# tomn681/Flow-Matching-and-Diffusion-Models

Measured on AMD Instinct MI355X. Metric: train images/sec + sampler steps/sec, LDCT 256x256 UNet at 1/2/4/8 MI355X, higher is better.
Workload: dtype bf16; 1 GPU; LDCT 2D 256x256 flow-matching train step (configs/flow_matching/ldct_flow_matching.json, EfficientUNetND 113M, concatenate conditioning) + 50-step FlowMatchEuler sampler; global_batch=8, per_gpu_batch=8, img=256, parallelism=dp1, hipgraph=True

## Files before the change

flow-matching-and-diffusion-models_amd/csrc/conv.hip:

```cpp
#include <cstdlib>
#include "halo_args.h"
#include "splitk_combine.h"

namespace {

struct KArgs {
  fmd_conv_desc d;
  fmd_gn_apply_desc g;
  int M;
  int T;
  int C;
  int nk1;
  int nk;
  int per_split;
  int ntp, ntc;
  int stats_rows;
  int par;
  int Mfull;
  int pack;
};

template <int BCO, int BPX, int WM, int WN, int BK, bool GNA = false>
__global__ __launch_bounds__(256, 2) void conv_igemm(const KArgs A) {
  constexpr int NT = 256;
// ... 352 lines not shown
#pragma unroll
      for (int kk = 0; kk < NB; ++kk) {
        const int k = kk;
        const int pi = (tid + 256 * (k0 + kk)) / CHT;
        const int p = min(px0 + pi, A.M - 1);
        vz[k] = *(const u32x4*)((const bf16r*)g.dz + (size_t)p * C + co);
        vx[k] = first ? *(const u32x4*)((const bf16r*)g.x0 + (size_t)p * C0 + co)
                      : *(const u32x4*)((const bf16r*)g.x1 + (size_t)p * C1 + (co - C0));
        old[k] = u32x4{0u, 0u, 0u, 0u};
        if (accf)
          old[k] = first ? *(const u32x4*)((const bf16r*)g.dx0 + (size_t)p * C0 + co)
                         : *(const u32x4*)((const bf16r*)g.dx1 + (size_t)p * C1 + (co - C0));
      }
#pragma unroll
      for (int k = 0; k < NB; ++k) {
        const int pi = (tid + 256 * (k0 + k)) / CHT;
        const int p = px0 + pi;
        if (p >= A.M) continue;
        const int n = p / HWo;
        const u32x4 ve = *(const u32x4*)(tile + pi * BCO + ((c16 ^ (pi & (CHT - 1))) * 8));
        bf16r* dst = first ? (bf16r*)g.dx0 + (size_t)p * C0 + co : (bf16r*)g.dx1 + (size_t)p * C1 + (co - C0);
        const float* pp = g.P + (size_t)n * C + co;
        const float* qq = g.Q + (size_t)n * C + co;
        const float* rr = g.R + (size_t)n * C + co;
        const f32x4 P0 = *(const f32x4*)pp, P1 = *(const f32x4*)(pp + 4);
        const f32x4 Q0 = *(const f32x4*)qq, Q1 = *(const f32x4*)(qq + 4);
        const f32x4 R0 = *(const f32x4*)rr, R1 = *(const f32x4*)(rr + 4);
        const float Pv[8] = {P0[0], P0[1], P0[2], P0[3], P1[0], P1[1], P1[2], P1[3]};
        const float Qv[8] = {Q0[0], Q0[1], Q0[2], Q0[3], Q1[0], Q1[1], Q1[2], Q1[3]};
        const float Rv[8] = {R0[0], R0[1], R0[2], R0[3], R1[0], R1[1], R1[2], R1[3]};
        u32x4 o;
#pragma unroll
        for (int e = 0; e < 4; ++e) {
          float lo = Pv[2 * e] * bf_lo(vz[k][e]) + Qv[2 * e] * bf_lo(vx[k][e]) + Rv[2 * e] + bf_lo(ve[e]);
          float hi = Pv[2 * e + 1] * bf_hi(vz[k][e]) + Qv[2 * e + 1] * bf_hi(vx[k][e]) + Rv[2 * e + 1] +
                     bf_hi(ve[e]);
          if (accf) { lo += bf_lo(old[k][e]); hi += bf_hi(old[k][e]); }
          o[e] = pack2(lo, hi);
        }
        *(u32x4*)dst = o;
      }
      }
    }
    return;
  }

  const bool stats = d.stats != nullptr;
  const bool dep = d.ep_a != nullptr;
  const bool hasx = d.ep_x0 != nullptr;
  float st1[TM][4], st2[TM][4];
#pragma unroll
  for (int i = 0; i < TM; ++i)
#pragma unroll
    for (int r = 0; r < 4; ++r) { st1[i][r] = 0.f; st2[i][r] = 0.f; }

#pragma unroll
  for (int i = 0; i < TM; ++i) {
    const int co = co0 + wm * (BCO / WM) + 16 * i + 4 * lq;
    if (co >= K) continue;
    const bool full = co + 3 < K;
    float bias[4] = {0.f, 0.f, 0.f, 0.f};
    if (d.bias) {
      for (int r = 0; r < 4; ++r) bias[r] = (co + r < K) ? d.bias[co + r] : 0.f;
    }
    if (d.bias2) {
      for (int r = 0; r < 4; ++r) bias[r] += (co + r < K) ? d.bias2[co + r] : 0.f;
    }
#pragma unroll
    for (int j = 0; j < TN; ++j) {
// ... 581 lines not shown
```

flow-matching-and-diffusion-models_amd/csrc/wgrad.hip:

```cpp
#include "common.h"
#include "../../include/fmdiff.h"

namespace {

constexpr int BCO = 128, BCI = 128, BKP = 32;

struct WArgs {
  fmd_wgrad_desc d;
  int M, T, C, ntc, nci, per_split, nsteps, ldy;
  int merged;
};

FMD_DEV int swz(int row) { return 4 * ((row & 3) | (((row >> 3) & 1) << 2)); }
FMD_DEV int lds_off(int row, int unit) { return row * 128 + 4 * (unit ^ swz(row)); }

FMD_DEV void wgrad_body(const WArgs& A, int bx, const int split, const int nsplit) {
  __shared__ __attribute__((aligned(16))) bf16r lds[2][2][BKP * 128];
  __shared__ float bsum[4][BCO];
  const fmd_wgrad_desc& d = A.d;
  const int tid = threadIdx.x, lane = tid & 63, wid = tid >> 6;
  const int wm = wid >> 1, wn = wid & 1;

  const int tco = bx % A.ntc; bx /= A.ntc;
  const int tci = bx % A.nci; bx /= A.nci;
// ... 406 lines not shown
    rc = (int)hipGetLastError();
  }
  if (rc) return rc;
  int nblk = 0;
  for (int j = 0; j < n; ++j) {
    const WArgs& A = G.a[j];
    const int lanes = 512 / (16 * A.T);
    G.gx[j] = max(1, min(G.nsplit[j], lanes));
    G.start[j] = nblk;
    int rows = A.d.K;
    if (G.nsplit[j] == 1) {
      G.gx[j] = lanes;
      rows = (A.d.K + lanes - 1) / lanes;
    }
    nblk += rows * ((A.C + RC - 1) / RC);
  }
  for (int j = n; j <= FMD_WGRAD_GROUP_MAX; ++j) G.start[j] = nblk;
  hipLaunchKernelGGL(wgrad_reduce2_group, dim3(nblk), dim3(512), 0, s, G);
  return (int)hipGetLastError();
}

extern "C" int fmd_wgrad(const fmd_wgrad_desc* d, fmd_stream_t stream) {
  hipStream_t s = (hipStream_t)stream;
  if (int rc = check_desc(d)) return rc;
  WArgs A = make_args(d);
  const int splits = d->splits > 1 ? d->splits : 1;
  int rc = d->force_generic ? 1 : fmd_wgrad_halo(d, stream);
  if (rc == 1) {
    dim3 grid(A.ntc * (A.merged ? A.nci : A.nci * A.T), splits);
    hipLaunchKernelGGL(wgrad_kernel, grid, dim3(256), 0, s, A);
    rc = (int)hipGetLastError();
  }
  if (rc) return rc;
  if (A.T > 27) return -4;
  if (A.C % 4 == 0) {
    const int sl = max(1, min(splits, 512 / (16 * A.T)));
    hipLaunchKernelGGL(wgrad_reduce2, dim3(d->K, (A.C + RC - 1) / RC), dim3(512), 0, s, A, splits, splits, 1, sl);
  } else {
    hipLaunchKernelGGL(wgrad_reduce, dim3(d->K, (A.C + RC - 1) / RC), dim3(256), 0, s, A, splits, splits, 1);
  }
  return (int)hipGetLastError();
}
```

flow-matching-and-diffusion-models_amd/fmdiff/_lib.py:

```python
from __future__ import annotations

import ctypes as C
import os

LIB_PATH = os.environ.get("FMD_LIB") or os.path.join(os.path.dirname(os.path.abspath(__file__)), "lib",
                                                     "libfmdiff_hip.so")

p = C.c_void_p
i32 = C.c_int32
i64 = C.c_int64
f32 = C.c_float
u32 = C.c_uint32


class ConvDesc(C.Structure):
    _fields_ = [
        ("N", i32), ("Hs", i32), ("Ws", i32), ("C0", i32), ("C1", i32), ("Ho", i32), ("Wo", i32), ("K", i32),
        ("ks", i32), ("stride", i32), ("pad", i32), ("upsample", i32), ("transposed", i32),
        ("src0", p), ("src1", p), ("pro_a", p), ("pro_b", p), ("pro_silu", i32), ("wgt", p),
        ("src2", p), ("src3", p), ("C2", i32), ("C3", i32), ("wgt2", p),
        ("bias", p), ("bias2", p), ("bias_nc", p), ("resid", p), ("out", p), ("out_f32", i32), ("accumulate", i32),
        ("stats", p), ("ep_x0", p), ("ep_x1", p), ("ep_C0", i32), ("ep_a", p), ("ep_b", p),
        ("ws", p), ("splits", i32), ("force_generic", i32), ("wgt_tiled", p), ("wgt2_tiled", p),
        ("Ds", i32), ("Do", i32), ("gout", p),
        ("fold_st0", p), ("fold_rows0", i32), ("fold_st1", p), ("fold_rows1", i32), ("fold_G", i32),
        ("fold_eps", f32), ("fold_gamma", p), ("fold_beta", p), ("fold_emb", p), ("fold_emb_stride", i32),
        ("tickets", p), ("n_tickets", i32), ("tickets_rows", i32),
    ]


class ConvPlan(C.Structure):
    _fields_ = [("kernel", i32), ("tile_rows", i32), ("bco", i32), ("bpx", i32), ("tickets", i32),
                ("combine_launch", i32), ("stats_rows", i32), ("fold", i32)]


CONV_IGEMM, CONV_HALO8, CONV_HALO9 = 1, 2, 3
CONV_TICKET_HALO, CONV_TICKET_IGEMM, CONV_WANT_STATS = 1, 2, 4


class WgradDesc(C.Structure):
    _fields_ = [
        ("N", i32), ("Hs", i32), ("Ws", i32), ("C0", i32), ("C1", i32), ("Ho", i32), ("Wo", i32), ("K", i32),
        ("ks", i32), ("stride", i32), ("pad", i32), ("upsample", i32),
        ("src0", p), ("src1", p), ("pro_a", p), ("pro_b", p), ("pro_silu", i32), ("dy", p), ("ldy", i32), ("dw", p), ("db", p),
        ("accumulate", i32), ("ws", p), ("splits", i32), ("force_generic", i32), ("Ds", i32), ("Do", i32),
    ]


class GnApplyDesc(C.Structure):
    _fields_ = [
        ("dz", p), ("x0", p), ("x1", p), ("C0", i32), ("P", p), ("Q", p), ("R", p),
        ("dx0", p), ("acc0", i32), ("dx1", p), ("acc1", i32),
    ]


class GnOutDesc(C.Structure):
    _fields_ = [("G", i32), ("eps", f32), ("gamma", p), ("beta", p), ("emb", p), ("emb_stride", i32),
                ("emb_mode", i32), ("silu", i32), ("a", p), ("b", p), ("mean_rstd", p), ("t", p)]


class ConvSmallDesc(C.Structure):
    _fields_ = [
        ("N", i32), ("Hs", i32), ("Ws", i32), ("C0", i32), ("C1", i32), ("Ho", i32), ("Wo", i32), ("K", i32),
        ("mode", i32), ("src0", p), ("src1", p), ("wgt", p), ("st0", p), ("rows0", i32), ("st1", p), ("rows1", i32),
        ("G", i32), ("eps", f32), ("gamma", p), ("beta", p), ("emb", p), ("emb_stride", i32), ("silu", i32),
        ("src2", p), ("src3", p), ("C2", i32), ("C3", i32), ("wgt2", p), ("bias", p), ("bias2", p), ("bias_nc", p),
        ("bias_nc_stride", i32), ("resid", p),
        ("out", p), ("stats", p), ("part", p), ("part_bytes", i64), ("tickets", p), ("n_tickets", i32), ("split", i32),
    ]


LINCOMB_MAX = 6


class LincombDesc(C.Structure):
    _fields_ = [("out", p), ("in_", p * LINCOMB_MAX), ("c", C.c_float * LINCOMB_MAX), ("nin", i32), ("n", i64)]


SCHED_NCOEF = 12


class SchedStepDesc(C.Structure):
    _fields_ = [("x", p), ("eps", p), ("ring", p * 4), ("last", p), ("coef", p), ("index", p), ("N", i32), ("Cx", i32),
                ("HW", i32), ("Kpad", i32), ("cond", p), ("Cc", i32), ("Cpad", i32), ("next", p)]


class GbJob(C.Structure):
    _fields_ = [("ws", p), ("dgamma", p), ("dbeta", p), ("N", i32), ("C", i32)]


GB_MAX = 64


class VqPlan(C.Structure):
    _fields_ = [("splits", i32), ("block_rows", i32), ("tile_codes", i32), ("codes_per_split", i32), ("Kpad", i32),
                ("Dpad", i32), ("finalize_rows", i32)]


SIGNATURES = {
    "fmd_conv": [C.POINTER(ConvDesc), p],
    "fmd_conv_plan": [C.POINTER(ConvDesc), i32, C.POINTER(ConvPlan)],
    "fmd_conv_halo": [C.POINTER(ConvDesc), p],
    "fmd_conv_gn_apply": [C.POINTER(ConvDesc), C.POINTER(GnApplyDesc), p],
    "fmd_conv_gn": [C.POINTER(ConvDesc), C.POINTER(GnOutDesc), p],
    "fmd_wgrad": [C.POINTER(WgradDesc), p],
    "fmd_wgrad_workspace": [C.POINTER(WgradDesc)],
    "fmd_wgrad_halo": [C.POINTER(WgradDesc), p],
    "fmd_wgrad_group": [C.POINTER(WgradDesc), i32, p],
    "fmd_wgrad_halo_group": [C.POINTER(WgradDesc), i32, p],
    "fmd_halo_tiled_size": [i32, i32, i32],
    "fmd_tile_weights_halo": [p, i32, i32, i32, p, p],
    "fmd_conv_s2d": [C.POINTER(ConvDesc), p],
    "fmd_conv_d2s": [C.POINTER(ConvDesc), p],
    "fmd_conv_small_plan": [C.POINTER(ConvSmallDesc)],
    "fmd_conv_small_split": [C.POINTER(ConvSmallDesc)],
    "fmd_conv_small": [C.POINTER(ConvSmallDesc), p],
    "fmd_s2d_tiled_size": [i32, i32, i32],
    "fmd_s2d_tile_weights": [p, i32, i32, i32, i32, p, p],
    "fmd_s2d_tiled_size_nd": [i32, i32, i32, i32, i32],
    "fmd_s2d_tile_weights_nd": [p, i32, i32, i32, i32, i32, p, p],
    "fmd_channel_stats": [p, p, p, i32, i32, i32, i32, i32, p, p],
    "fmd_stats_fold": [p, i64, i32, i32, p, p],
    "fmd_gn_prep": [p, i32, p, i32, i32, i32, i32, i32, i32, f32, p, p, p, i32, i32, p, p, p, p],
    "fmd_gn_bwd_prep": [p, i32, i32, i32, i32, i32, p, p, p, p, i32, i32, p, p, p, p, p, p, i32, p, i32, p, p],
    "fmd_gn_apply_fwd": [p, p, i32, i32, i64, i32, p, p, i32, p, p],
    "fmd_gn_fused_apply": [p, p, i32, i32, i32, i32, i32, f32, p, p, p, i32, i32, i32, p, p, p, p, p],
    "fmd_dropout_apply": [p, i32, i64, i32, f32, p, u32, p, p, p, p, p],
    "fmd_gn_gb_fold": [p, i32, p],
    "fmd_lincomb": [C.POINTER(LincombDesc), p],
    "fmd_sched_step": [C.POINTER(SchedStepDesc), p],
    "fmd_halo_set_min_workgroups": [i32],
    "fmd_halo_set_th8_max_workgroups": [i32],
    "fmd_halo_set_th4_max_workgroups": [i32],
    "fmd_conv_gn_set_block_channels": [i32],
    "fmd_gn_bwd_apply": [p, p, p, i32, i32, i64, i32, p, p, p, p, p, i32, p, i32, p],
    "fmd_prep_weights": [p, i32, i32, i32, i32, i32, i32, p, p],
    "fmd_prep_weights_t": [p, i32, i32, i32, i32, i32, i32, p, p],
    "fmd_prep_weights_batch": [p, i32, i32, p],
    "fmd_prep_weights_batch_cubic": [p, i32, i32, p],
    "fmd_nchw_to_nhwc": [p, i32, i32, i32, i32, p, p],
    "fmd_nhwc_to_nchw": [p, i32, i32, i32, i32, i32, p, p],
    "fmd_sum_pool2": [p, i32, i32, i32, i32, p, i32, p],
# ... 96 lines not shown
```

flow-matching-and-diffusion-models_amd/fmdiff/runtime/engine.py:

```python
from __future__ import annotations

import math
import weakref
from typing import List, Optional, Tuple

import torch

from . import ops, tuning
from ..nn.blocks.attention import DiffusersAttentionND, SpatialCrossAttention, SpatialSelfAttention
from ..nn.blocks.residual import ResBlockND
from ..nn.ops.convolution import ConvND
from ..nn.ops.upsampling import DownsampleND, UpsampleND
from ..nn.params import Conv, Identity

BF16 = torch.bfloat16
F32 = torch.float32
CPAD = 8
HALO_BK = 32
MAT3D = bool(tuning.get("MAT3D"))
DEPTH_HALO = bool(tuning.get("DEPTH_HALO"))
S2D_HALO = bool(tuning.get("S2D_HALO"))
S2D_3D = S2D_HALO and bool(tuning.get("S2D_3D"))
POINT_1X1 = bool(tuning.get("POINT_1X1"))
SMALL_ATTN = bool(tuning.get("SMALL_ATTN"))
# ... 546 lines not shown
            a2, b2, mr2 = ops.gn_prep(hst, None, N, HW, Cout, 0, g2.num_groups, g2.eps, g2.weight, g2.bias)
        pf2 = (dict(st0=hst, groups=g2.num_groups, eps=g2.eps, gamma=g2.weight, beta=g2.bias, emb=eo if ss else None,
                    emb_stride=es if ss else 0) if a2 is None and t2 is None else None)
        sk = m.skip_connection
        kw = {}
        if isinstance(sk, Identity):
            if x1 is not None:
                raise ValueError("identity skip with concatenated input")
            kw["resid"] = x0.t
        else:
            _check_conv(sk.conv, 1, 1, 0)
        if mat2 and not halo2:
            halo2 = self._halo_ok(N, sp, Cout, Cout)
        if not isinstance(sk, Identity):
            s2, s2t = self._wts(sk.conv.weight, 0, halo2)
            kw.update(src2=x0.t, src3=x1.t if x1 else None, wgt2=s2, wgt2_tiled=s2t, bias2=sk.conv.bias)
        point2 = POINT_1X1 and sp == (1, 1) and c2.weight.dim() == 4 and not halo2
        w2, w2t = (self.wc.get(self.wc.center(c2.weight), 0), None) if point2 else self._wts(c2.weight, 0, halo2)
        if point2:
            kw.update(ks=1, pad=0)
        if mat2 and t2 is None:
            t2 = ops.gn_apply_fwd(h, None, a2, b2)
        if drop:
            ops.dropout_apply(t2, drop, seed, salt, out=t2)
        gg2 = (torch.empty_like(h) if keep_g and t2 is None and halo2 and not point2 and Cout % HALO_BK == 0
               else None)
        out, ost = ops.conv(t2 if t2 is not None else h, Cout, w2,
                            pro=None if (t2 is not None or pf2 is not None) else (a2, b2, True), pro_fold=pf2,
                            bias=c2.bias, want_stats="free", wgt_tiled=w2t, gout=gg2, **kw)
        o = Act(out, ost)
        if ctx.tape is None:
            return o

        def bwd():
            dy = o.grad

            def wg2():
                if t2 is not None or gg2 is not None:
                    ops.wgrad(t2 if t2 is not None else gg2, dy, c2.weight.grad, db=c2.bias.grad)
                else:
                    ops.wgrad(h, dy, c2.weight.grad, pro=(a2, b2, True), db=c2.bias.grad)
                if not isinstance(sk, Identity):
                    ops.wgrad(x0.t, dy, sk.conv.weight.grad, src1=x1.t if x1 else None, ks=1, pad=0,
                              db=sk.conv.bias.grad)
            self._wg(wg2, N * HW)
            extra = dy if isinstance(sk, Identity) else None
            if drop:
                dd, _ = self.dgrad3x3(c2.weight, dy, Cout, sp)
                dz2 = ops.dropout_apply(dd, drop, seed, salt, ep=(h, a2, b2), out=dd)
                s2 = ops.channel_stats(dz2, y=(h, None, Cout))
            else:
                dz2, s2 = self.dgrad3x3(c2.weight, dy, Cout, sp, ep=(h, None, a2, b2), want_stats=True)
            if slot is not None:
                demb, ds_ = ctx.demb_all[:, slot[0]:slot[0] + slot[1]], self.gl.total
            elif eo is not None:
                demb = torch.empty_like(eo)
                ds_ = demb.shape[1]
            else:
                demb, ds_ = None, 0
            if ss:
                P2, Q2, R2 = ops.gn_bwd_prep(s2, N, HW, Cout, g2.num_groups, mr2, g2.weight, g2.bias, g2.weight.grad,
                                             g2.bias.grad, emb=eo, emb_stride=es, emb_mode=1, demb=demb,
                                             demb_stride=ds_)
            elif add:
                P2, Q2, R2 = ops.gn_bwd_prep(s2, N, HW, Cout, g2.num_groups, mr2, g2.weight, g2.bias, g2.weight.grad,
                                             g2.bias.grad, emb_mode=2, demb=demb, demb_stride=ds_, fwd=hst)
            else:
                P2, Q2, R2 = ops.gn_bwd_prep(s2, N, HW, Cout, g2.num_groups, mr2, g2.weight, g2.bias, g2.weight.grad,
                                             g2.bias.grad)
            dh = torch.empty_like(h)
            ops.gn_bwd_apply(dz2, h, None, P2, Q2, R2, None, dh, 0)
            del dz2
            if t1 is not None or gg1 is not None:
                self._wg(lambda: ops.wgrad(t1 if t1 is not None else gg1, dh, c1.weight.grad, db=c1.bias.grad),
                         N * HW)
            else:
                self._wg(lambda: ops.wgrad(x0.t, dh, c1.weight.grad, src1=x1.t if x1 else None, pro=(a1, b1, True),
                                           db=c1.bias.grad), N * HW)
            dz1, s1 = self.dgrad3x3(c1.weight, dh, Cin, sp, ep=(x0.t, x1.t if x1 else None, a1, b1),
                                    want_stats=True)
            P1, Q1, R1 = ops.gn_bwd_prep(s1, N, HW, Cin, g1.num_groups, mr1, g1.weight, g1.bias, g1.weight.grad,
                                         g1.bias.grad)
            d0, acc0 = _gdest(x0)
            d1, acc1 = _gdest(x1)
            if isinstance(sk, Identity):
                ops.gn_bwd_apply(dz1, x0.t, x1.t if x1 else None, P1, Q1, R1, extra, d0, acc0, d1, acc1)
            else:
                ops.conv1x1_gn_apply(dy, self.wc.get(sk.conv.weight, 1), dz1, x0.t, x1.t if x1 else None,
                                     P1, Q1, R1, d0, acc0, d1, acc1)
            if (ss or add) and slot is None:
                ops.linear_bwd(ctx.emb, el.weight, demb, el.weight.grad, el.bias.grad, dx=ctx.demb, dx_acc=True,
                               in_silu=m.emb_activation_before_proj)
        ctx.tape.append(bwd)
        return o

    def _res_block_small(self, m: ResBlockND, x0: Act, x1: Optional[Act], eo, es, ss: bool, add: bool):
        N, H, W, C0 = x0.t.shape
        C1 = x1.C if x1 is not None else 0
        Cout = m.out_channels
        c1, c2 = m.conv1.conv, m.conv2.conv
        if c1.weight.dim() != 4 or c2.weight.dim() != 4:
            return None
        _check_conv(c1, 3, 1, 1)
        _check_conv(c2, 3, 1, 1)
        point = POINT_1X1 and (H, W) == (1, 1)
        mode = "point" if point else "s1"
        g1, g2 = m.norm1, m.norm2
        sk = m.skip_connection
        ident = isinstance(sk, Identity)
        if ident and x1 is not None:
            raise ValueError("identity skip with concatenated input")
        if not ident:
            _check_conv(sk.conv, 1, 1, 0)
        rows = 64 if (H * W) % 64 == 0 else H * W

        def probe(a):
            return a.stats if a.stats is not None else ops.Stats(None, rows)
        gn1 = dict(st0=probe(x0), st1=probe(x1) if x1 is not None else None, groups=g1.num_groups, eps=g1.eps)
        gn2 = dict(st0=ops.Stats(None, rows), groups=g2.num_groups, eps=g2.eps, emb=eo if ss else None,
# ... 514 lines not shown
```

flow-matching-and-diffusion-models_amd/fmdiff/runtime/ops.py:

```python
from __future__ import annotations

import ctypes as C
from dataclasses import dataclass
from typing import Optional, Tuple

import torch

from .. import _lib
from . import tuning, wgrad_plan
from .._lib import ConvDesc, GnApplyDesc, GnOutDesc, WgradDesc

BF16 = torch.bfloat16
F32 = torch.float32
NUM_CU = 256


def _p(t: Optional[torch.Tensor]):
    return None if t is None else t.data_ptr()


def stream():
    return C.c_void_p(torch.cuda.current_stream().cuda_stream)


def _need_cuda(t: torch.Tensor, what: str):
    if t.device.type != "cuda":
        raise RuntimeError(f"{what}: fmdiff HIP kernels need ROCm device tensors (got {t.device}); "
                           "there is no CPU path")


@dataclass
class Stats:
    slab: torch.Tensor
    rows: int


def channel_stats(x: torch.Tensor, rows: Optional[int] = None, y: Tuple = None) -> Stats:
    N, Cc = x.shape[0], x.shape[-1]
    HW = x[0, ..., 0].numel()
    if rows is None:
        rows = 64 if HW % 64 == 0 else HW
    slab = torch.empty((N * HW // rows, Cc, 2), device=x.device, dtype=F32)
    y0, y1, C0 = (None, None, Cc) if y is None else y
# ... 755 lines not shown
        self.prev, _wgrad_queue = _wgrad_queue, self.queue

    def __exit__(self, *exc):
        global _wgrad_queue
        _wgrad_queue = self.prev


def wgrad(src0, dy, dw, *, src1=None, ks=3, stride=1, pad=1, upsample=False, pro=None, db=None, accumulate=True,
          splits=None, dy_offset=0, force_generic=False, immediate=False):
    q = _wgrad_queue
    if dw.dim() == 3 and dw.shape[2] > 1 and src0.dim() == 4:
        full = torch.zeros((*dw.shape[:2], ks, ks), device=dw.device, dtype=F32)
        wgrad(src0, dy, full, src1=src1, ks=ks, stride=stride, pad=pad, upsample=upsample, pro=pro, db=db,
              accumulate=accumulate, splits=splits, dy_offset=dy_offset, force_generic=force_generic, immediate=True)
        col = full[..., (ks - 1) // 2]
        if accumulate:
            dw.add_(col)
        else:
            dw.copy_(col)
        return
    job = wgrad_job(src0, dy, dw, src1=src1, ks=ks, stride=stride, pad=pad, upsample=upsample, pro=pro, db=db,
                    accumulate=accumulate, dy_offset=dy_offset, force_generic=force_generic)
    if q is not None:
        if (not immediate and splits is None and src0.dim() == 4
                and job.shape.pixels <= WGRAD_GROUP_MAX_PIX):
            q.push(job)
            return
        q.flush()
    job.d.splits = job.single_splits() if splits is None else splits
    ws = _wgrad_workspace([job])
    _lib.call("fmd_wgrad", C.byref(job.d), stream())


def prep_weights(w: torch.Tensor, mode: int, Kpad: Optional[int] = None, Cpad: Optional[int] = None, out=None):
    K, Cc = w.shape[0], w.shape[1]
    ks = w.shape[2] if w.dim() >= 4 else 1
    Kpad = Kpad or K
    Cpad = Cpad or Cc
    if w.dim() == 5:
        T = ks ** 3
        shape = (Kpad, T, Cpad) if mode == 0 else (Cpad, T, Kpad)
        if out is None:
            out = torch.empty(shape, device=w.device, dtype=BF16)
        _lib.call("fmd_prep_weights_t", _p(w.contiguous()), K, Cc, T, mode, Kpad, Cpad, _p(out), stream())
        return out
    T = 16 if mode == 2 else ks * ks
    shape = (Kpad, T, Cpad) if mode == 0 else (Cpad, T, Kpad)
    if out is None:
        out = torch.empty(shape, device=w.device, dtype=BF16)
    _lib.call("fmd_prep_weights", _p(w.contiguous()), K, Cc, ks, mode, Kpad, Cpad, _p(out), stream())
    return out


def tile_weights(wk: torch.Tensor, out=None):
    R, T, Cc = wk.shape
    n = int(_lib.lib().fmd_halo_tiled_size(R, T, Cc))
    if out is None:
        out = torch.empty((n,), device=wk.device, dtype=BF16)
    _lib.call("fmd_tile_weights_halo", _p(wk), R, T, Cc, _p(out), stream())
    return out


def nchw_to_nhwc(x: torch.Tensor, Cpad: Optional[int] = None) -> torch.Tensor:
    _need_cuda(x, "nchw_to_nhwc")
    x = x.contiguous().float()
    N, Cc = x.shape[:2]
# ... 788 lines not shown
```

flow-matching-and-diffusion-models_amd/fmdiff/runtime/tuning.py:

```python
from __future__ import annotations

import os

TABLE = {
    "MAT3D": (1, "3-D: materialise the GN+SiLU operand of depth-tap halo convs once (0: fused prologue + G side "
                 "output)"),
    "DEPTH_HALO": (1, "3x3x3 stride-1 convs on the halo kernel with (depth tap, channel block) chunks"),
    "S2D_HALO": (1, "stride-2 3x3 forwards / nearest-x2 data gradients on the space-to-depth halo kernel"),
    "S2D_3D": (1, "3-D: the same stride-2 modes with the depth taps as chunks (0: generic implicit GEMM, and the "
                  "nearest-x2 data gradient at full resolution + 2x2x2 box sum)"),
    "WGRAD_S2D": (1, "2-D stride-2 3x3 weight gradients on the halo weight-gradient kernel (space-to-depth planes as "
                     "chunks; 0: the generic weight-gradient kernel).  2-D only: 3-D stride-2 weight gradients always "
                     "run on the generic kernel (fmd_wgrad_halo rejects them)"),
    "POINT_1X1": (1, "ResBlock 3x3 convs on 1x1 images as their centre tap"),
    "GN_FUSED": (1, "small levels: GroupNorm statistics + affine + SiLU operand in one launch"),
    "CONV_GN": (1, "split-K conv1 -> GroupNorm-2 in the split combine (fmd_conv_gn)"),
    "HALO_FOLD": (1, "forward only: the GroupNorm affine folded in the halo conv's prologue (no gn_prep launch)"),
    "HALO_FOLD_MAX_ROWS": (64, "... where the statistics slab has at most this many rows per image"),
    "HALO_TICKET": (1, "split-K halo convs combined inside the launch (arrival tickets) instead of a combine launch"),
    "SPLIT_TICKET": (0, "... and split-K implicit-GEMM convs on whole tiles likewise (off: their 8-16 parts make one "
                        "workgroup's serial combine slower than the combine launch -- train 369.6 -> 363.5 img/s)"),
    "CAPTURE_STREAM": (1, "graph captures on a side stream whose in-launch-combine workspace exists beforehand"),
    "SMALL_ATTN": (1, "forward-only small levels: attention's qkv (GroupNorm folded) and output projections on fmd_conv_small"),
    "SMALL_CONV": (1, "forward-only small levels: one launch per conv with the GroupNorm folded in (fmd_conv_small)"),
    "SMALL_CONV_MAX_HW": (256, "fmd_conv_small only on outputs of at most this many pixels per image"),
    "SMALL_CONV_MAX_WORK": (65536, "... and output pixels per image x input channels at most this (16^2 x 256: config D's "
                                   "16^2 level, not config B's 512-channel one; DESIGN.md round 6)"),
    "SMALL_CONV_SPLIT": (0, "fmd_conv_small reduction parts combined in-launch: 0 plan's choice, 1 none, 2..16 forced"),
    "CONV_GN_MIN_BLOCKS": (128, "fmd_conv_gn only from this many combine blocks up"),
    "CONV_GN_CB": (4, "fmd_conv_gn combine block channels (4, 8, 16, 32, 64; at least one group)"),
    "STATS_FOLD_MIN": (4096, "statistics slabs with at least this many rows per image are folded first"),
    "SPLIT_MIN_STEPS": (2, "generic conv split-K: at least this many K-steps per split"),
    "SPLIT_CU_MULT": (2, "generic conv split-K: target workgroups per CU"),
    "SPLIT_CAP": (64, "generic conv split-K: most splits"),
    "HALO_SPLIT_WG": (256, "halo conv split-K: target workgroups"),
    "HALO_MIN_CHUNKS": (2, "halo conv split-K: at least this many 32-channel chunks per split"),
    "HALO_SPLIT_CAP": (16, "halo conv split-K: most splits"),
    "HALO_MIN_WG": (32, "halo conv only from this many workgroups (tiles x cout tiles x splits) up"),
    "HALO_TH8_MAX_WG": (1024, "halo conv: 8-row tiles for grids of fewer 16-row workgroups than this (0: never)"),
    "HALO_TH4_MAX_WG": (512, "halo conv: 4-row tiles for 8-row grids of fewer workgroups than this (0: never)"),
    "WGRAD_MIN_STEPS": (8, "generic weight gradient: at least this many 32-pixel steps per split"),
    "WGRAD_CU_MULT": (4, "generic weight gradient: target workgroups per CU"),
    "WGRAD_HALO_WG": (0, "halo weight gradient: target workgroups (0 = one per CU)"),
    "WGRAD_SLAB_MB": (96, "halo weight gradient: split-K slab cap (MB)"),
    "WGRAD_GEN_SLAB_MB": (48, "generic weight gradient: split-K slab cap (MB)"),
    "WGRAD_GROUP": (1, "the engine defers a level's weight gradients and runs them as grouped launches "
                       "(fmd_wgrad_group) with the group plan's splits (0: each at once, alone)"),
    "WGRAD_GROUP_MAX_PIX": (131072, "... only on output grids of at most this many pixels (N x H x W; config B: "
                                    "the 128^2 level and below); larger levels run each weight gradient at once, "
                                    "its operands still in the Infinity Cache (DESIGN.md round 7: the 256^2 level "
                                    "measured no gain grouped)"),
    "WGRAD_GROUP_SPLITS": (0, "grouped weight gradients: 0 = the group plan's splits, 1 = every job's own ungrouped "
                              "splits (bit-identical to WGRAD_GROUP=0; parity bisection)"),
}

RETIRED = sorted({f"FMD_{k}" for k in TABLE} | {
    "FMD_HALO9", "FMD_HALO10", "FMD_WGRAD9", "FMD_WGRAD_REDUCE", "FMD_WGRAD_REDUCE1", "FMD_WGRAD_PIPE", "FMD_WGRAD_KS",
    "FMD_SPLITK_FUSE", "FMD_WRED_BATCH", "FMD_SIDE_WGRAD", "FMD_MAT_PRO", "FMD_GOUT", "FMD_CONV_LOG", "FMD_X"})


def check_environment(env=None) -> None:
    env = os.environ if env is None else env
    stale = [k for k in RETIRED if k in env]
    if stale:
        raise ValueError(f"retired environment switch(es) {', '.join(stale)}: the runtime no longer reads them; use "
                         f"FMD_TUNE=\"NAME=value,...\" with the names of fmdiff/runtime/tuning.py TABLE")


check_environment()
_over = {}
for _item in filter(None, (s.strip() for s in os.environ.get("FMD_TUNE", "").split(","))):
    _k, _, _v = _item.partition("=")
    if _k not in TABLE or not _v:
        raise ValueError(f"FMD_TUNE: unknown or empty setting {_item!r} (known: {', '.join(TABLE)})")
    _over[_k] = int(_v)


def get(name: str) -> int:
    return _over.get(name, TABLE[name][0])


def overridden(name: str) -> bool:
    return name in _over
```

include/fmdiff.h:

```cpp
#ifndef FMDIFF_H
#define FMDIFF_H
#include <stdint.h>

#ifdef __cplusplus
extern "C" {
#endif

typedef void* fmd_stream_t;

typedef struct fmd_conv_desc {
  int32_t N, Hs, Ws;
  int32_t C0, C1;
  int32_t Ho, Wo, K;
  int32_t ks, stride, pad;
  int32_t upsample;
  int32_t transposed;
  const void* src0;
  const void* src1;
  const float* pro_a;
  const float* pro_b;
  int32_t pro_silu;
  const void* wgt;
  const void* src2;
  const void* src3;
// ... 137 lines not shown
int fmd_conv_small_split(const fmd_conv_small_desc* d);
int fmd_conv_small(const fmd_conv_small_desc* d, fmd_stream_t s);

int fmd_head_fwd(const void* h, int32_t N, int32_t D, int32_t H, int32_t W, int32_t C, const float* pro_a,
                 const float* pro_b, const float* w, const float* bias, int32_t K, float* out, fmd_stream_t s);
int fmd_head_dgrad(const void* dpred, const float* w, int32_t K, const void* h, const float* pro_a, const float* pro_b,
                   int32_t N, int32_t D, int32_t H, int32_t W, int32_t C, void* dz, float* stats, fmd_stream_t s);
int64_t fmd_head_wgrad_workspace(int32_t N, int32_t D, int32_t H, int32_t W, int32_t C, int32_t K);
int fmd_head_wgrad(const void* dpred, int32_t K, const void* h, const float* pro_a, const float* pro_b, int32_t N,
                   int32_t D, int32_t H, int32_t W, int32_t C, float* dw, float* db, float* ws, fmd_stream_t s);

typedef struct fmd_wgrad_desc {
  int32_t N, Hs, Ws, C0, C1, Ho, Wo, K, ks, stride, pad, upsample;
  const void* src0; const void* src1;
  const float* pro_a; const float* pro_b; int32_t pro_silu;
  const void* dy;
  int32_t ldy;
  float* dw;
  float* db;
  int32_t accumulate;
  float* ws;
  int32_t splits;
  int32_t force_generic;
  int32_t Ds, Do;
} fmd_wgrad_desc;

int fmd_wgrad(const fmd_wgrad_desc* d, fmd_stream_t s);
int fmd_wgrad_halo(const fmd_wgrad_desc* d, fmd_stream_t s);
int64_t fmd_wgrad_workspace(const fmd_wgrad_desc* d);

#define FMD_WGRAD_GROUP_MAX 16
int fmd_wgrad_group(const fmd_wgrad_desc* descs, int32_t n, fmd_stream_t s);
int fmd_wgrad_halo_group(const fmd_wgrad_desc* descs, int32_t n, fmd_stream_t s);

int fmd_channel_stats(const void* x, const void* y0, const void* y1, int32_t C0, int32_t N, int32_t HW, int32_t C,
                      int32_t rows, float* out , fmd_stream_t s);
int fmd_stats_fold(const float* slab, int64_t rows_total, int32_t C, int32_t fold, float* out, fmd_stream_t s);
int fmd_gn_prep(const float* st0, int32_t rows0, const float* st1, int32_t rows1, int32_t N, int32_t HW,
                int32_t C0, int32_t C1, int32_t G, float eps, const float* gamma, const float* beta,
                const float* emb, int32_t emb_stride, int32_t emb_mode ,
                float* a, float* b, float* mean_rstd, fmd_stream_t s);
int fmd_gn_bwd_prep(const float* s12, int32_t rows, int32_t N, int32_t HW, int32_t C, int32_t G,
                    const float* mean_rstd, const float* gamma, const float* beta, const float* emb,
                    int32_t emb_stride, int32_t emb_mode, float* P, float* Q, float* R,
                    float* dgamma, float* dbeta, float* demb, int32_t demb_stride, const float* fwd_st,
                    int32_t fwd_rows, float* ws , fmd_stream_t s);
#define FMD_GB_MAX 64
typedef struct {
  const float* ws;
  float* dgamma;
  float* dbeta;
  int32_t N, C;
} fmd_gb_job;
int fmd_gn_gb_fold(const fmd_gb_job* jobs, int32_t njobs, fmd_stream_t s);
int fmd_gn_fused_apply(const void* x0, const void* x1, int32_t C0, int32_t C1, int32_t N, int32_t HW, int32_t G,
                       float eps, const float* gamma, const float* beta, const float* emb, int32_t emb_stride,
                       int32_t emb_mode, int32_t silu, float* a, float* b, float* mean_rstd, void* t,
                       fmd_stream_t s);
int fmd_gn_apply_fwd(const void* x0, const void* x1, int32_t C0, int32_t C1, int64_t M, int32_t HW,
                     const float* a, const float* b, int32_t silu, void* t, fmd_stream_t s);

int fmd_dropout_apply(const void* x, int32_t C, int64_t M, int32_t HW, float p, const int32_t* seed, uint32_t salt,
                      const void* ep_x, const float* ep_a, const float* ep_b, void* y, fmd_stream_t s);
int fmd_gn_bwd_apply(const void* dz, const void* x0, const void* x1, int32_t C0, int32_t C1, int64_t M,
                     int32_t HW, const float* P, const float* Q, const float* R, const void* extra,
                     void* dx0, int32_t acc0, void* dx1, int32_t acc1, fmd_stream_t s);
// ... 164 lines not shown
```

Before: 371.6 train images/s.

## Fuse ResBlock skip-conv weight, bias and data gradients into one backward kernel

Adds a skip_bwd kernel that, in a single pass over pixel tiles, computes the 1x1 skip conv data gradient, fuses it with the GroupNorm backward apply, and accumulates the skip weight and bias gradients into per-group slabs. A split-out wgrad combine reduces those slabs. This replaces the separate conv1x1_gn_apply and ks=1 wgrad launches, so dy and x are read once instead of twice. It is enabled by default only for levels with enough tiles per group, and adds workspace plus a new kernel. The existing gn-apply epilogue also gains an explicit fma.

```diff
diff --git a/flow-matching-and-diffusion-models_amd/csrc/conv.hip b/flow-matching-and-diffusion-models_amd/csrc/conv.hip
--- a/flow-matching-and-diffusion-models_amd/csrc/conv.hip
+++ b/flow-matching-and-diffusion-models_amd/csrc/conv.hip
@@ -408,9 +408,10 @@
         u32x4 o;
 #pragma unroll
         for (int e = 0; e < 4; ++e) {
-          float lo = Pv[2 * e] * bf_lo(vz[k][e]) + Qv[2 * e] * bf_lo(vx[k][e]) + Rv[2 * e] + bf_lo(ve[e]);
-          float hi = Pv[2 * e + 1] * bf_hi(vz[k][e]) + Qv[2 * e + 1] * bf_hi(vx[k][e]) + Rv[2 * e + 1] +
-                     bf_hi(ve[e]);
+          float lo = __builtin_fmaf(Pv[2 * e], bf_lo(vz[k][e]), Qv[2 * e] * bf_lo(vx[k][e])) + Rv[2 * e] +
+                     bf_lo(ve[e]);
+          float hi = __builtin_fmaf(Pv[2 * e + 1], bf_hi(vz[k][e]), Qv[2 * e + 1] * bf_hi(vx[k][e])) +
+                     Rv[2 * e + 1] + bf_hi(ve[e]);
           if (accf) { lo += bf_lo(old[k][e]); hi += bf_hi(old[k][e]); }
           o[e] = pack2(lo, hi);
         }
diff --git a/flow-matching-and-diffusion-models_amd/csrc/skip_bwd.hip b/flow-matching-and-diffusion-models_amd/csrc/skip_bwd.hip
--- /dev/null
+++ b/flow-matching-and-diffusion-models_amd/csrc/skip_bwd.hip
@@ -0,0 +1,317 @@
+#include "common.h"
+#include "../../include/fmdiff.h"
+
+namespace {
+
+constexpr int KD = 128, CT = 128, BPX = 64, NT = 256;
+
+struct SArgs {
+  fmd_skip_bwd_desc d;
+  int M, C, HW;
+  int ntp, ntc;
+  int G;
+  int nsl;
+  int xcd;
+};
+
+FMD_DEV int swz(int row) { return 4 * ((row & 3) | (((row >> 3) & 1) << 2)); }
+FMD_DEV int toff(int row, int unit) { return row * 128 + 4 * (unit ^ swz(row)); }
+
+__global__ __launch_bounds__(NT, 2) void skip_bwd_kernel(const SArgs A) {
+  __shared__ __attribute__((aligned(16))) bf16r ldsW[CT * KD];
+  __shared__ __attribute__((aligned(16))) bf16r ldsY[BPX * KD];
+  __shared__ __attribute__((aligned(16))) bf16r ldsX[BPX * CT];
+  const fmd_skip_bwd_desc& d = A.d;
+  const fmd_gn_apply_desc& g = d.g;
+  const int tid = threadIdx.x, lane = tid & 63, wid = tid >> 6;
+  const int wm = wid >> 1, wn = wid & 1;
+  const int l16 = lane & 15, lq = lane >> 4;
+
+  const int b = blockIdx.x;
+  int ct, grp;
+  if (A.xcd) {
+    const int k = b >> 3;
+    ct = k % A.ntc;
+    grp = (k / A.ntc) * 8 + (b & 7);
+  } else {
+    ct = b % A.ntc;
+    grp = b / A.ntc;
+  }
+  if (grp >= A.ntp) return;
+
+  const int C = A.C, C0 = g.C0, C1 = C - g.C0;
+  const int chunk = tid & 15, rb = tid >> 4;
+  const int co = ct * CT + chunk * 8;
+  const bool c_ok = co < C;
+  const bool first = co < C0;
+  const int accf = first ? g.acc0 : g.acc1;
+  const bool do_bias = d.db && ct == 0;
+  const bf16r* __restrict__ dy = (const bf16r*)d.dy;
+  const bf16r* __restrict__ xs = first ? (const bf16r*)g.x0 + co : (const bf16r*)g.x1 + (co - C0);
+  bf16r* __restrict__ dxs = first ? (bf16r*)g.dx0 + co : (bf16r*)g.dx1 + (co - C0);
+  const int ldx = first ? C0 : C1;
+  const bf16r* __restrict__ dzs = (const bf16r*)g.dz + co;
+
+  {
+    const bf16r* w = (const bf16r*)d.wgt_t;
+#pragma unroll
+    for (int j = 0; j < CT / 16; ++j) {
+      const int r = rb + 16 * j;
+      u32x4 v = {0u, 0u, 0u, 0u};
+      if (ct * CT + r < C) v = *(const u32x4*)(w + (size_t)(ct * CT + r) * KD + chunk * 8);
+      *(u32x4*)(ldsW + r * KD + 8 * (chunk ^ (r & 15))) = v;
+    }
+  }
+
+  u32x4 ry[4], rx[4], vz[4], old[4];
+  const u32x4 zero4 = {0u, 0u, 0u, 0u};
+  auto load_yx = [&](int t) {
+#pragma unroll
+    for (int j = 0; j < 4; ++j) {
+      const int p = t * BPX + rb + 16 * j;
+      const bool ok = p < A.M;
+      ry[j] = ok ? *(const u32x4*)(dy + (size_t)p * KD + chunk * 8) : zero4;
+      rx[j] = ok && c_ok ? *(const u32x4*)(xs + (size_t)p * ldx) : zero4;
+    }
+  };
+  auto load_zo = [&](int t) {
+#pragma unroll
+    for (int j = 0; j < 4; ++j) {
+      const int p = t * BPX + rb + 16 * j;
+      const bool ok = p < A.M && c_ok;
+      vz[j] = ok ? *(const u32x4*)(dzs + (size_t)p * C) : zero4;
+      old[j] = ok && accf ? *(const u32x4*)(dxs + (size_t)p * ldx) : zero4;
+    }
+  };
+
+  f32x4 accw[4][4];
+#pragma unroll
+  for (int i = 0; i < 4; ++i)
+#pragma unroll
+    for (int j = 0; j < 4; ++j) accw[i][j] = f32x4{0.f, 0.f, 0.f, 0.f};
+  float bacc[8];
+#pragma unroll
+  for (int e = 0; e < 8; ++e) bacc[e] = 0.f;
+
+  const int lg = lane >> 4, q = (lane >> 2) & 3, pp = lane & 3;
+  auto frag = [&](const bf16r* t, int st, int col0) -> bf16x8 {
+    const s16x4 lo = ds_read_tr16(t + toff(32 * st + 8 * lg + q, col0 / 4 + pp));
+    const s16x4 hi = ds_read_tr16(t + toff(32 * st + 8 * lg + 4 + q, col0 / 4 + pp));
+    typedef __attribute__((ext_vector_type(8))) short s16x8;
+    s16x8 v = {lo[0], lo[1], lo[2], lo[3], hi[0], hi[1], hi[2], hi[3]};
+    return __builtin_bit_cast(bf16x8, v);
+  };
+
+  load_yx(grp);
+  load_zo(grp);
+#pragma unroll 1
+  for (int t = grp; t < A.ntp; t += A.G) {
+    const bool nxt = t + A.G < A.ntp;
+#pragma unroll
+    for (int j = 0; j < 4; ++j) {
+      const int r = rb + 16 * j;
+      *(u32x4*)(ldsY + toff(r, 2 * chunk)) = ry[j];
+      *(u32x4*)(ldsX + toff(r, 2 * chunk)) = rx[j];
+    }
+    if (do_bias) {
+#pragma unroll
+      for (int j = 0; j < 4; ++j)
+#pragma unroll
+        for (int e = 0; e < 4; ++e) {
+          bacc[2 * e] += bf_lo(ry[j][e]);
+          bacc[2 * e + 1] += bf_hi(ry[j][e]);
+        }
+    }
+    __syncthreads();
+    if (nxt) load_yx(t + A.G);
+
+    f32x4 acc[4][2];
+#pragma unroll
+    for (int i = 0; i < 4; ++i)
+#pragma unroll
+      for (int j = 0; j < 2; ++j) acc[i][j] = f32x4{0.f, 0.f, 0.f, 0.f};
+#pragma unroll
+    for (int kk = 0; kk < KD / 32; ++kk) {
+      const int kc = 4 * kk + lq;
+      bf16x8 af[4], bfr[2];
+#pragma unroll
+      for (int i = 0; i < 4; ++i) {
+        const int r = wm * 64 + 16 * i + l16;
+        af[i] = *(const bf16x8*)(ldsW + r * KD + 8 * (kc ^ (r & 15)));
+      }
+#pragma unroll
+      for (int j = 0; j < 2; ++j) {
+        const int r = wn * 32 + 16 * j + l16;
+        bfr[j] = *(const bf16x8*)(ldsY + toff(r, 2 * kc));
+      }
+#pragma unroll
+      for (int i = 0; i < 4; ++i)
+#pragma unroll
+        for (int j = 0; j < 2; ++j) acc[i][j] = mfma16(af[i], bfr[j], acc[i][j]);
+    }
+
+#pragma unroll
+    for (int st = 0; st < BPX / 32; ++st) {
+      bf16x8 af[4], bfr[4];
+#pragma unroll
+      for (int i = 0; i < 4; ++i) af[i] = frag(ldsY, st, wm * 64 + 16 * i);
+#pragma unroll
+      for (int j = 0; j < 4; ++j) bfr[j] = frag(ldsX, st, wn * 64 + 16 * j);
+#pragma unroll
+      for (int i = 0; i < 4; ++i)
+#pragma unroll
+        for (int j = 0; j < 4; ++j) accw[i][j] = mfma16(af[i], bfr[j], accw[i][j]);
+    }
+    __syncthreads();
+
+#pragma unroll
+    for (int i = 0; i < 4; ++i) {
+      const int cl = wm * 64 + 16 * i + 4 * lq;
+#pragma unroll
+      for (int j = 0; j < 2; ++j) {
+        const int pi = wn * 32 + 16 * j + l16;
+        u32x2 o;
+        o[0] = pack2(acc[i][j][0], acc[i][j][1]);
+        o[1] = pack2(acc[i][j][2], acc[i][j][3]);
+        *(u32x2*)(ldsY + pi * CT + (((cl >> 3) ^ (pi & 15)) * 8) + (cl & 7)) = o;
+      }
+    }
+    __syncthreads();
+
+    if (c_ok) {
+#pragma unroll
+      for (int k = 0; k < 4; ++k) {
+        const int pi = rb + 16 * k;
+        const int p = t * BPX + pi;
+        if (p >= A.M) continue;
+        const int n = p / A.HW;
+        const u32x4 ve = *(const u32x4*)(ldsY + pi * CT + ((chunk ^ (pi & 15)) * 8));
+        const u32x4 vx = *(const u32x4*)(ldsX + toff(pi, 2 * chunk));
+        const float* pq = g.P + (size_t)n * C + co;
+        const float* qq = g.Q + (size_t)n * C + co;
+        const float* rr = g.R + (size_t)n * C + co;
+        const f32x4 P0 = *(const f32x4*)pq, P1 = *(const f32x4*)(pq + 4);
+        const f32x4 Q0 = *(const f32x4*)qq, Q1 = *(const f32x4*)(qq + 4);
+        const f32x4 R0 = *(const f32x4*)rr, R1 = *(const f32x4*)(rr + 4);
+        const float Pv[8] = {P0[0], P0[1], P0[2], P0[3], P1[0], P1[1], P1[2], P1[3]};
+        const float Qv[8] = {Q0[0], Q0[1], Q0[2], Q0[3], Q1[0], Q1[1], Q1[2], Q1[3]};
+        const float Rv[8] = {R0[0], R0[1], R0[2], R0[3], R1[0], R1[1], R1[2], R1[3]};
+        u32x4 o;
+#pragma unroll
+        for (int e = 0; e < 4; ++e) {
+          float lo = __builtin_fmaf(Pv[2 * e], bf_lo(vz[k][e]), Qv[2 * e] * bf_lo(vx[e])) + Rv[2 * e] + bf_lo(ve[e]);
+          float hi = __builtin_fmaf(Pv[2 * e + 1], bf_hi(vz[k][e]), Qv[2 * e + 1] * bf_hi(vx[e])) + Rv[2 * e + 1] +
+                     bf_hi(ve[e]);
+          if (accf) { lo += bf_lo(old[k][e]); hi += bf_hi(old[k][e]); }
+          o[e] = pack2(lo, hi);
+        }
+        *(u32x4*)(dxs + (size_t)p * ldx) = o;
+      }
+    }
+    if (nxt) load_zo(t + A.G);
+    __syncthreads();
+  }
+
+  const size_t per = (size_t)KD * C;
+  float* ws = d.ws + (size_t)grp * per;
+#pragma unroll
+  for (int i = 0; i < 4; ++i) {
+#pragma unroll
+    for (int j = 0; j < 4; ++j) {
+      const int ci = ct * CT + wn * 64 + 16 * j + l16;
+      if (ci >= C) continue;
+#pragma unroll
+      for (int r = 0; r < 4; ++r) {
+        const int k = wm * 64 + 16 * i + 4 * lq + r;
+        ws[(size_t)k * C + ci] = accw[i][j][r];
+      }
+    }
+  }
+  if (do_bias) {
+    float* bsum = (float*)ldsY;
+#pragma unroll
+    for (int e = 0; e < 8; ++e) {
+      float v = bacc[e];
+      v += __shfl_xor(v, 16, 64);
+      v += __shfl_xor(v, 32, 64);
+      bacc[e] = v;
+    }
+    if (lane < 16) {
+#pragma unroll
+      for (int e = 0; e < 8; ++e) bsum[wid * KD + chunk * 8 + e] = bacc[e];
+    }
+    __syncthreads();
+    if (tid < KD) {
+      float* wb = d.ws + (size_t)A.nsl * per + (size_t)grp * KD;
+      wb[tid] = bsum[tid] + bsum[KD + tid] + bsum[2 * KD + tid] + bsum[3 * KD + tid];
+    }
+  }
+}
+
+int decide(const fmd_skip_bwd_desc* d, SArgs* A, fmd_skip_bwd_plan_t* p) {
+  *p = fmd_skip_bwd_plan_t{};
+  const int64_t M64 = (int64_t)d->N * d->HW;
+  const int C = d->C0 + d->C1;
+  if (d->Kd != KD || d->N < 1 || d->HW < 1 || (d->C0 % 8) || (d->C1 % 8) || d->C0 < 8) return 1;
+  if (C <= 64) return 1;
+  if (M64 > (int64_t)1 << 30) return 1;
+  const int M = (int)M64;
+  const int ntp = (M + BPX - 1) / BPX, ntc = (C + CT - 1) / CT;
+  const int ncu = d->num_cu > 0 ? d->num_cu : 256;
+  int G;
+  if (d->groups > 0) {
+    G = d->groups;
+  } else {
+    G = 2 * ncu / ntc;
+    if (G < 1) G = 1;
+    if (G > ntp) G = ntp;
+    if (G >= 8) G -= G % 8;
+    if ((int64_t)ntp < (int64_t)d->min_tiles * G) return 1;
+  }
+  if ((int64_t)G * ntc > 65535) return 1;
+  const int nsl = G < ntp ? G : ntp;
+  p->taken = 1;
+  p->c_tile = CT;
+  p->workgroups = G * ntc;
+  p->slabs = nsl;
+  p->ws_floats = (int64_t)nsl * ((int64_t)KD * C + KD);
+  if (A) {
+    A->d = *d;
+    A->M = M;
+    A->C = C;
+    A->HW = d->HW;
+    A->ntp = ntp;
+    A->ntc = ntc;
+    A->G = G;
+    A->nsl = nsl;
+    A->xcd = G % 8 == 0;
+  }
+  return 0;
+}
+
+}
+
+extern "C" int fmd_skip_bwd_plan(const fmd_skip_bwd_desc* d, fmd_skip_bwd_plan_t* out) {
+  return decide(d, nullptr, out);
+}
+
+extern "C" int fmd_skip_bwd(const fmd_skip_bwd_desc* d, fmd_stream_t stream) {
+  SArgs A;
+  fmd_skip_bwd_plan_t p;
+  if (decide(d, &A, &p)) return -1;
+  const fmd_gn_apply_desc& g = d->g;
+  if (!d->dy || !d->wgt_t || !d->dw || !d->ws) return -2;
+  if (!g.dz || !g.x0 || !g.P || !g.Q || !g.R || !g.dx0 || g.C0 != d->C0) return -7;
+  if (d->C1 && (!g.x1 || !g.dx1)) return -7;
+  hipStream_t s = (hipStream_t)stream;
+  hipLaunchKernelGGL(skip_bwd_kernel, dim3(p.workgroups), dim3(NT), 0, s, A);
+  int rc = (int)hipGetLastError();
+  if (rc) return rc;
+  fmd_wgrad_desc w = {};
+  w.N = d->N; w.Hs = w.Ho = d->HW; w.Ws = w.Wo = 1;
+  w.C0 = d->C0 + d->C1; w.K = KD;
+  w.ks = 1; w.stride = 1;
+  w.dw = d->dw; w.db = d->db; w.accumulate = d->accumulate;
+  w.ws = d->ws; w.splits = p.slabs;
+  return fmd_wgrad_combine(&w, stream);
+}
diff --git a/flow-matching-and-diffusion-models_amd/csrc/wgrad.hip b/flow-matching-and-diffusion-models_amd/csrc/wgrad.hip
--- a/flow-matching-and-diffusion-models_amd/csrc/wgrad.hip
+++ b/flow-matching-and-diffusion-models_amd/csrc/wgrad.hip
@@ -462,6 +462,14 @@
     rc = (int)hipGetLastError();
   }
   if (rc) return rc;
+  return fmd_wgrad_combine(d, stream);
+}
+
+extern "C" int fmd_wgrad_combine(const fmd_wgrad_desc* d, fmd_stream_t stream) {
+  hipStream_t s = (hipStream_t)stream;
+  if (int rc = check_desc(d)) return rc;
+  WArgs A = make_args(d);
+  const int splits = d->splits > 1 ? d->splits : 1;
   if (A.T > 27) return -4;
   if (A.C % 4 == 0) {
     const int sl = max(1, min(splits, 512 / (16 * A.T)));
diff --git a/flow-matching-and-diffusion-models_amd/fmdiff/_lib.py b/flow-matching-and-diffusion-models_amd/fmdiff/_lib.py
--- a/flow-matching-and-diffusion-models_amd/fmdiff/_lib.py
+++ b/flow-matching-and-diffusion-models_amd/fmdiff/_lib.py
@@ -54,6 +54,16 @@
     ]
 
 
+class SkipBwdDesc(C.Structure):
+    _fields_ = [("N", i32), ("HW", i32), ("C0", i32), ("C1", i32), ("Kd", i32), ("dy", p), ("wgt_t", p),
+                ("g", GnApplyDesc), ("dw", p), ("db", p), ("accumulate", i32), ("ws", p), ("groups", i32),
+                ("num_cu", i32), ("min_tiles", i32)]
+
+
+class SkipBwdPlan(C.Structure):
+    _fields_ = [("taken", i32), ("c_tile", i32), ("workgroups", i32), ("slabs", i32), ("ws_floats", i64)]
+
+
 class GnOutDesc(C.Structure):
     _fields_ = [("G", i32), ("eps", f32), ("gamma", p), ("beta", p), ("emb", p), ("emb_stride", i32),
                 ("emb_mode", i32), ("silu", i32), ("a", p), ("b", p), ("mean_rstd", p), ("t", p)]
@@ -108,6 +118,9 @@
     "fmd_wgrad_halo": [C.POINTER(WgradDesc), p],
     "fmd_wgrad_group": [C.POINTER(WgradDesc), i32, p],
     "fmd_wgrad_halo_group": [C.POINTER(WgradDesc), i32, p],
+    "fmd_wgrad_combine": [C.POINTER(WgradDesc), p],
+    "fmd_skip_bwd_plan": [C.POINTER(SkipBwdDesc), C.POINTER(SkipBwdPlan)],
+    "fmd_skip_bwd": [C.POINTER(SkipBwdDesc), p],
     "fmd_halo_tiled_size": [i32, i32, i32],
     "fmd_tile_weights_halo": [p, i32, i32, i32, p, p],
     "fmd_conv_s2d": [C.POINTER(ConvDesc), p],
diff --git a/flow-matching-and-diffusion-models_amd/fmdiff/runtime/engine.py b/flow-matching-and-diffusion-models_amd/fmdiff/runtime/engine.py
--- a/flow-matching-and-diffusion-models_amd/fmdiff/runtime/engine.py
+++ b/flow-matching-and-diffusion-models_amd/fmdiff/runtime/engine.py
@@ -602,6 +602,9 @@
         if ctx.tape is None:
             return o
 
+        skip_fused = (not isinstance(sk, Identity) and sk.conv.bias is not None
+                      and ops.skip_bwd_plan(N, HW, C0, C1, Cout) is not None)
+
         def bwd():
             dy = o.grad
 
@@ -610,7 +613,7 @@
                     ops.wgrad(t2 if t2 is not None else gg2, dy, c2.weight.grad, db=c2.bias.grad)
                 else:
                     ops.wgrad(h, dy, c2.weight.grad, pro=(a2, b2, True), db=c2.bias.grad)
-                if not isinstance(sk, Identity):
+                if not isinstance(sk, Identity) and not skip_fused:
                     ops.wgrad(x0.t, dy, sk.conv.weight.grad, src1=x1.t if x1 else None, ks=1, pad=0,
                               db=sk.conv.bias.grad)
             self._wg(wg2, N * HW)
@@ -655,6 +658,10 @@
             d1, acc1 = _gdest(x1)
             if isinstance(sk, Identity):
                 ops.gn_bwd_apply(dz1, x0.t, x1.t if x1 else None, P1, Q1, R1, extra, d0, acc0, d1, acc1)
+            elif skip_fused:
+                if not ops.skip_bwd(dy, self.wc.get(sk.conv.weight, 1), dz1, x0.t, x1.t if x1 else None, P1, Q1, R1,
+                                    d0, acc0, d1, acc1, sk.conv.weight.grad, sk.conv.bias.grad):
+                    raise RuntimeError("skip_bwd: the plan that took this block at trace time now refuses it")
             else:
                 ops.conv1x1_gn_apply(dy, self.wc.get(sk.conv.weight, 1), dz1, x0.t, x1.t if x1 else None,
                                      P1, Q1, R1, d0, acc0, d1, acc1)
diff --git a/flow-matching-and-diffusion-models_amd/fmdiff/runtime/ops.py b/flow-matching-and-diffusion-models_amd/fmdiff/runtime/ops.py
--- a/flow-matching-and-diffusion-models_amd/fmdiff/runtime/ops.py
+++ b/flow-matching-and-diffusion-models_amd/fmdiff/runtime/ops.py
@@ -8,7 +8,7 @@
 
 from .. import _lib
 from . import tuning, wgrad_plan
-from .._lib import ConvDesc, GnApplyDesc, GnOutDesc, WgradDesc
+from .._lib import ConvDesc, GnApplyDesc, GnOutDesc, SkipBwdDesc, SkipBwdPlan, WgradDesc
 
 BF16 = torch.bfloat16
 F32 = torch.float32
@@ -830,6 +830,59 @@
     _lib.call("fmd_wgrad", C.byref(job.d), stream())
 
 
+SKIP_BWD = bool(tuning.get("SKIP_BWD"))
+SKIP_BWD_MIN_TILES = tuning.get("SKIP_BWD_MIN_TILES")
+
+
+class _SkipWs:
+    __slots__ = ("d", "device")
+
+    def __init__(self, Kd, C0, C1, slabs, device):
+        self.d = WgradDesc()
+        self.d.K, self.d.C0, self.d.C1, self.d.ks, self.d.splits = Kd, C0, C1, 1, slabs
+        self.device = device
+
+
+def _skip_bwd_desc(N, HW, C0, C1, Kd, groups=0, min_tiles=None) -> SkipBwdDesc:
+    d = SkipBwdDesc()
+    d.N, d.HW, d.C0, d.C1, d.Kd, d.groups, d.num_cu = N, HW, C0, C1, Kd, groups, NUM_CU
+    d.min_tiles = SKIP_BWD_MIN_TILES if min_tiles is None else min_tiles
+    return d
+
+
+def skip_bwd_plan(N, HW, C0, C1, Kd, groups=0, min_tiles=None) -> Optional[SkipBwdPlan]:
+    if not SKIP_BWD:
+        return None
+    p = SkipBwdPlan()
+    rc = _lib.lib().fmd_skip_bwd_plan(C.byref(_skip_bwd_desc(N, HW, C0, C1, Kd, groups, min_tiles)), C.byref(p))
+    return p if rc == 0 and p.taken else None
+
+
+def skip_bwd(dy, wgt_t, dz, x0, x1, P, Q, R, dx0, acc0, dx1, acc1, dw, db, accumulate=True, groups=0,
+             min_tiles=None) -> bool:
+    _need_cuda(dy, "skip_bwd")
+    N, Kd = dy.shape[0], dy.shape[-1]
+    HW = dy[0, ..., 0].numel()
+    C0 = x0.shape[-1]
+    C1 = x1.shape[-1] if x1 is not None else 0
+    plan = skip_bwd_plan(N, HW, C0, C1, Kd, groups, min_tiles)
+    if plan is None:
+        return False
+    d = _skip_bwd_desc(N, HW, C0, C1, Kd, groups, min_tiles)
+    d.dy, d.wgt_t = _p(dy), _p(wgt_t)
+    d.g.dz, d.g.x0, d.g.x1, d.g.C0 = _p(dz), _p(x0), _p(x1), C0
+    d.g.P, d.g.Q, d.g.R = _p(P), _p(Q), _p(R)
+    d.g.dx0, d.g.acc0, d.g.dx1, d.g.acc1 = _p(dx0), int(acc0), _p(dx1), int(acc1)
+    d.dw, d.db, d.accumulate = _p(dw), _p(db), int(accumulate)
+    job = _SkipWs(Kd, C0, C1, plan.slabs, dy.device)
+    ws = _wgrad_workspace([job])
+    if ws.numel() < plan.ws_floats:
+        raise RuntimeError("skip_bwd: workspace smaller than the plan's")
+    d.ws = job.d.ws
+    _lib.call("fmd_skip_bwd", C.byref(d), stream())
+    return True
+
+
 def prep_weights(w: torch.Tensor, mode: int, Kpad: Optional[int] = None, Cpad: Optional[int] = None, out=None):
     K, Cc = w.shape[0], w.shape[1]
     ks = w.shape[2] if w.dim() >= 4 else 1
diff --git a/flow-matching-and-diffusion-models_amd/fmdiff/runtime/tuning.py b/flow-matching-and-diffusion-models_amd/fmdiff/runtime/tuning.py
--- a/flow-matching-and-diffusion-models_amd/fmdiff/runtime/tuning.py
+++ b/flow-matching-and-diffusion-models_amd/fmdiff/runtime/tuning.py
@@ -50,6 +50,10 @@
                                     "the 128^2 level and below); larger levels run each weight gradient at once, "
                                     "its operands still in the Infinity Cache (DESIGN.md round 7: the 256^2 level "
                                     "measured no gain grouped)"),
+    "SKIP_BWD": (1, "ResBlock skip conv: weight, bias and data gradient in the GroupNorm-1 backward pass "
+                    "(fmd_skip_bwd) where its plan takes the block (0: fmd_conv_gn_apply + the ks=1 weight gradient)"),
+    "SKIP_BWD_MIN_TILES": (8, "... only with at least this many 64-pixel tiles per pixel group (config B at batch 8: "
+                              "the 128^2 level and above, the levels traced faster fused; DESIGN.md round 17)"),
     "WGRAD_GROUP_SPLITS": (0, "grouped weight gradients: 0 = the group plan's splits, 1 = every job's own ungrouped "
                               "splits (bit-identical to WGRAD_GROUP=0; parity bisection)"),
 }
diff --git a/include/fmdiff.h b/include/fmdiff.h
--- a/include/fmdiff.h
+++ b/include/fmdiff.h
@@ -193,6 +193,31 @@
 #define FMD_WGRAD_GROUP_MAX 16
 int fmd_wgrad_group(const fmd_wgrad_desc* descs, int32_t n, fmd_stream_t s);
 int fmd_wgrad_halo_group(const fmd_wgrad_desc* descs, int32_t n, fmd_stream_t s);
+int fmd_wgrad_combine(const fmd_wgrad_desc* d, fmd_stream_t s);
+
+typedef struct fmd_skip_bwd_desc {
+  int32_t N, HW;
+  int32_t C0, C1, Kd;
+  const void* dy;
+  const void* wgt_t;
+  fmd_gn_apply_desc g;
+  float* dw;
+  float* db;
+  int32_t accumulate;
+  float* ws;
+  int32_t groups;
+  int32_t num_cu;
+  int32_t min_tiles;
+} fmd_skip_bwd_desc;
+typedef struct fmd_skip_bwd_plan_t {
+  int32_t taken;
+  int32_t c_tile;
+  int32_t workgroups;
+  int32_t slabs;
+  int64_t ws_floats;
+} fmd_skip_bwd_plan_t;
+int fmd_skip_bwd_plan(const fmd_skip_bwd_desc* d, fmd_skip_bwd_plan_t* out);
+int fmd_skip_bwd(const fmd_skip_bwd_desc* d, fmd_stream_t s);
 
 int fmd_channel_stats(const void* x, const void* y0, const void* y1, int32_t C0, int32_t N, int32_t HW, int32_t C,
                       int32_t rows, float* out , fmd_stream_t s);
```

New measurement: 382.1 train images/s, median of 6. 2.8% higher.
